# ShenhanQian/GaussianAvatars

Hardware: AMD Instinct MI355X
Metric: frames/sec fwd+bwd @100k SH-3 splats 802x550 (higher is better)
Workload: dtype f32; 1 GPU; BASELINE configs[2]: 100000 mesh-bound SH-3 splats (synthetic stand-in for media/306), 802x550 (HxW), select_mesh_by_timestep + render + L1-vs-white + backward, no optimiser step; splats=100000, width=550, height=802, sh_degree=3, scene=ellipsoid, splat_order=morton (io.spatial_sort: the loaders' default), num_rendered=2322054, num_binned=1851307, tile_culling=True, binding=fused, parallelism=one process, one GPU, 300 frames in turn; no collective

## Files before the change

gaussianavatars_amd/csrc/gsr_api.hip:

```cpp
#include <hip/hip_runtime.h>

#include <atomic>
#include <chrono>
#include <cstdarg>
#include <cstdio>
#include <cstdlib>
#include <cstring>
#include <map>
#include <mutex>
#include <tuple>
#include <thread>
#include <vector>

#include "gsr_device.h"


namespace {

thread_local char g_err[512] = "";

int fail(int code, const char* fmt, ...)
{
    va_list ap;
    va_start(ap, fmt);
// ... 488 lines not shown
    uint32_t* qpos = (uint32_t*)(b + bl.qpos);
    uint32_t* qcount = (uint32_t*)(b + bl.qcount);
    uint32_t* qstart = (uint32_t*)(b + bl.qstart);
    const bool write_lists = settings->tile_culling == 0 || settings->tile_culling == 2;
    uint32_t* qlist = (uint32_t*)(b + bl.qlist);

    if (prod) {
        const uint32_t nb = (uint32_t)bl.nb, chunks = (uint32_t)bl.chunks;
        const int Q = 4 * tiles;
        uint32_t* bcount = (uint32_t*)(b + bl.bcount);
        uint32_t* bstart = (uint32_t*)(b + bl.bstart);
        uint32_t* bcursor = (uint32_t*)(b + bl.bcursor);
        uint32_t* border = (uint32_t*)(b + bl.border);
        unsigned long long* dkeys = (unsigned long long*)(b + bl.dkeys);
        unsigned long long* dtmp = (unsigned long long*)(b + bl.dtmp);
        uint32_t* order = (uint32_t*)(b + bl.order);
        const uint32_t* brec_rect = (const uint32_t*)(g + gl.brec);
        {
            TIMED(GSR_K_DEPTH_SORT, stream);
            const int dblocks = pblocks < GSR_BIN_BLOCKS ? pblocks : GSR_BIN_BLOCKS;
            uint32_t* bhist = (uint32_t*)(b + bl.bhist);
            hipLaunchKernelGGL(gsr::k_dbucket, dim3(dblocks), dim3(256), (size_t)nb * 4, stream, P, brec_rect, (const float*)pa.depths, hdr, nb,
                               bcount, bhist);
            hipLaunchKernelGGL(gsr::k_dscan, dim3(1), dim3(1024), 0, stream, nb, (const uint32_t*)bcount, bstart, bcursor, border, hdr);
            hipLaunchKernelGGL(gsr::k_dscatter, dim3(dblocks), dim3(256), (size_t)nb * 4, stream, P, brec_rect, (const float*)pa.depths,
                               (const gsr::BinHeader*)hdr, nb, (const uint32_t*)bstart, bcursor, dkeys, (const uint32_t*)bhist);
            hipLaunchKernelGGL((gsr::k_dsort<GSR_SORT_SMALL_KEYS, 256>), dim3(nb), dim3(256), 0, stream, 0u, 0xFFFFFFFFu,
                               (const uint32_t*)border, (const uint32_t*)bcount, (const uint32_t*)bstart, dkeys, dtmp, order);
            KERNEL_CHECK("depth sort", stream, dbg);
        }
        gsr::QBinArgs qa;
        qa.Q = Q; qa.gx = gx; qa.chunks = chunks;
        qa.qmask = (unsigned long long*)(b + bl.qmask);
        qa.hdr = hdr; qa.brec = (const float4*)(g + gl.brec); qa.order = order;
        qa.qhist = (uint32_t*)(b + bl.qhist); qa.qprefix = (const uint32_t*)(b + bl.qprefix); qa.qstart = qstart; qa.qpos = qpos;
        qa.capacity = cap;
        const size_t count_lds = (((size_t)Q + 3) / 4) * 4;
        const size_t walk_lds = (size_t)Q * 4;
        if (walk_lds > 48 * 1024)
            if (int rc = ensure_dynamic_lds((const void*)gsr::k_qscatter, (size_t)walk_lds)) return rc;
        const int walk_blocks = (int)chunks;
        {
            TIMED(GSR_K_QCOUNT, stream);
            hipLaunchKernelGGL(gsr::k_qcount, dim3(walk_blocks), dim3(256), count_lds, stream, qa);
            KERNEL_CHECK("k_qcount", stream, dbg);
        }
        {
            TIMED(GSR_K_QSCAN, stream);
            hipLaunchKernelGGL(gsr::k_qscan, dim3(((Q + 3) / 4 + 31) / 32), dim3(1024), 0, stream, Q, chunks, (const uint8_t*)(b + bl.qhist),
                               (uint32_t*)(b + bl.qprefix), qcount);
            hipLaunchKernelGGL(gsr::k_qscan_glob, dim3(1), dim3(1024), 0, stream, tiles, (const uint32_t*)qcount, qstart, tile_order, hdr,
                               slot_dev, seq, post_cap);
            KERNEL_CHECK("k_qscan", stream, dbg);
        }
        {
            TIMED(GSR_K_QSCATTER, stream);
            hipLaunchKernelGGL(gsr::k_qscatter, dim3(walk_blocks), dim3(64), walk_lds, stream, qa);
            KERNEL_CHECK("k_qscatter", stream, dbg);
        }
    } else if (rankp) {
        const uint32_t nb = (uint32_t)bl.nb;
        const int bin_blocks = pblocks < GSR_RANK_BLOCKS ? pblocks : GSR_RANK_BLOCKS;
        const bool direct = gsr::rank_direct(gx, tiles);
        uint32_t* const chunk_bounds = reinterpret_cast<uint32_t*>((uint4*)(b + bl.pstat) + 5 * (size_t)pblocks);
        const size_t hist_bytes = direct ? 0 : (size_t)tiles * sizeof(uint32_t);
        const size_t count_lds = (size_t)nb * 4 + (direct ? 0 : (size_t)(gx + 1) * (size_t)(gy + 1) * sizeof(uint32_t));
        if (count_lds > 48 * 1024) {
            if (int rc = ensure_dynamic_lds((const void*)gsr::k_rcount, (size_t)count_lds)) return rc;
        }
        const bool one_band_lds = (int)bl.nbands <= 1;
        const size_t stage_bytes = GSR_RSCATTER_STAGE_BYTES(one_band_lds), hist_al = (hist_bytes + 15) & ~(size_t)15;
        static const bool balanced_on = [] { const char* e = getenv("GSR_RSCATTER_BALANCED"); return !(e && e[0] == '0'); }();
        const bool balanced = balanced_on && hist_al + stage_bytes + 20 * 1024 <= 160 * 1024;
        const int stage_off = balanced ? (int)hist_al : -1;
        const size_t scatter_lds = balanced ? hist_al + stage_bytes : hist_bytes;
        if (scatter_lds > 48 * 1024)
        {
            if (int rc = ensure_dynamic_lds((const void*)gsr::k_rsort_rscatter, scatter_lds)) return rc;
            if (int rc = ensure_dynamic_lds((const void*)gsr::k_rscatter<8>, scatter_lds)) return rc;
        }
        uint32_t* block_hist = (uint32_t*)(b + bl.block_hist);
        uint32_t* bcount = (uint32_t*)(b + bl.bcount);
        uint32_t* bstart = (uint32_t*)(b + bl.bstart);
        uint32_t* bcursor = (uint32_t*)(b + bl.bcursor);
        uint32_t* bhist = (uint32_t*)(b + bl.bhist);
        unsigned long long* dkeys = (unsigned long long*)(b + bl.dkeys);
        unsigned long long* dtmp = (unsigned long long*)(b + bl.dtmp);
        uint32_t* rank = (uint32_t*)(b + bl.rank);
        uint2* ranks = (uint2*)(b + bl.ranks);
        const int nbands = (int)bl.nbands;
        const float inv_band_rows = 1.0f / (float)bl.band_rows;
        uint2* obs = nbands > 1 ? (uint2*)(b + bl.obs) : nullptr;
        uint32_t* bandcnt = (uint32_t*)(b + bl.bandcnt);
        const uint32_t nwc = (uint32_t)(((size_t)P + GSR_RANK_BAND_CHUNK - 1) / GSR_RANK_BAND_CHUNK);
        gsr::BandTables bt;
        bt.nbands = (uint32_t)nbands;
        bt.inv_band_rows = inv_band_rows;
        bt.over = (const uint32_t*)(b + bl.rank_over);
        ushort4* srect = (ushort4*)(b + bl.srect);
        uint32_t* tile_start = (uint32_t*)(b + bl.tile_start);
        uint32_t* tile_cursor = (uint32_t*)(b + bl.tile_cursor);
        uint2* ranges = (uint2*)(b + bl.ranges);
        if (pblocks > 0) {
            TIMED(GSR_K_COUNT, stream);
            hipLaunchKernelGGL(gsr::k_rcount, dim3(bin_blocks), dim3(GSR_RANK_BIN_THREADS), count_lds, stream, rank_ilv, P, gx, tiles,
                               pblocks, nb, (const ushort4*)srect, (const uint32_t*)pa.tiles_touched,
                               (const float*)pa.depths, (const uint4*)pa.pstat, tile_count, rect_total, block_hist, bcount, bhist, hdr, chunk_bounds);
            KERNEL_CHECK("k_rcount", stream, dbg);
        }
        const bool one_band = nbands <= 1;
        {
            TIMED(GSR_K_DEPTH_SORT, stream);
            gsr::TileScanArgs ts;
            ts.tiles = tiles; ts.tile_count = tile_count; ts.tile_start = tile_start; ts.tile_cursor = tile_cursor; ts.ranges = ranges;
            ts.tile_order = tile_order; ts.tdesc = (uint4*)(b + bl.tdesc); ts.total_dev = total_dev; ts.mailbox = slot_dev; ts.seq = seq;
            ts.post_capacity = post_cap;
            ts.hdr = pblocks > 0 ? hdr : nullptr;
            hipLaunchKernelGGL(gsr::k_rdscatter, dim3((pblocks > 0 ? bin_blocks : 0) + 1), dim3(GSR_RANK_BIN_THREADS), (size_t)nb * 4, stream, rank_ilv, P, nb,
                               (const ushort4*)srect, (const float*)pa.depths, hdr, (const uint32_t*)bcount, bstart, bcursor, dkeys, (const uint32_t*)bhist, ts,
                               (const uint32_t*)chunk_bounds);
            KERNEL_CHECK("k_rdscatter", stream, dbg);
            if (!one_band && pblocks > 0) {
                hipLaunchKernelGGL(gsr::k_rdsort, dim3(nb), dim3(256), 0, stream, (const uint32_t*)bcount, (const uint32_t*)bstart, dkeys, dtmp, rank, obs,
                                   (const ushort4*)srect, (int)bl.band_rows);
                KERNEL_CHECK("k_rdsort", stream, dbg);
                const uint32_t wgs = (nwc + 3u) / 4u;
                hipLaunchKernelGGL(gsr::k_band_count, dim3(wgs), dim3(256), 0, stream, (const gsr::BinHeader*)hdr, (const uint2*)obs,
                                   (uint32_t)nbands, nwc, bandcnt);
                hipLaunchKernelGGL(gsr::k_band_scan, dim3(nbands), dim3(1024), 0, stream, hdr, nwc, bandcnt);
                hipLaunchKernelGGL(gsr::k_band_rank, dim3(wgs), dim3(256), 0, stream, (const gsr::BinHeader*)hdr, (const uint2*)obs,
                                   (uint32_t)nbands, nwc, (const uint32_t*)bandcnt, (uint4*)rank, (uint32_t*)(b + bl.rank_over));
                KERNEL_CHECK("k_band_rank", stream, dbg);
            }
        }
        if (pblocks > 0) {
            TIMED(GSR_K_SCATTER, stream);
            if (one_band) {
                hipLaunchKernelGGL(gsr::k_rsort_rscatter, dim3(bin_blocks + nb), dim3(GSR_RANK_BIN_THREADS), scatter_lds, stream, rank_ilv, bin_blocks, P, gx, tiles,
                                   (const ushort4*)srect, (const float4*)pa.sspan, (const uint32_t*)tile_start, tile_cursor, (uint32_t*)ranks, cap,
                                   (const unsigned long long*)total_dev, (const uint32_t*)block_hist, (const uint32_t*)bcount, (const uint32_t*)bstart,
                                   dkeys, dtmp, rank, stage_off, (const uint32_t*)chunk_bounds);
                KERNEL_CHECK("k_rsort_rscatter", stream, dbg);
            } else {
                hipLaunchKernelGGL(gsr::k_rscatter<8>, dim3(bin_blocks), dim3(GSR_RANK_BIN_THREADS), scatter_lds, stream, rank_ilv, P, gx, tiles, bt,
                                   (const ushort4*)srect, (const uint32_t*)rank, (const float4*)pa.sspan, (const uint32_t*)tile_start, tile_cursor, ranks, cap,
                                   (const unsigned long long*)total_dev, (const uint32_t*)block_hist, stage_off, (const uint32_t*)chunk_bounds);
                KERNEL_CHECK("k_rscatter", stream, dbg);
            }
        }
        {
            TIMED(GSR_K_TILE_SORT, stream);
            const size_t space = (size_t)P < (size_t)GSR_RANK_MAX_SPLATS ? (size_t)P : (size_t)GSR_RANK_MAX_SPLATS;
            const uint32_t words = (uint32_t)((space + 2047) / 2048) * 64u;
            hipLaunchKernelGGL(gsr::k_tile_rank, dim3(tiles), dim3(GSR_RANK_TILE_THREADS), (size_t)words * 6, stream, words, gx, nbands,
                               inv_band_rows, (const uint4*)(b + bl.tdesc), (const uint2*)ranks, one_band ? (const uint32_t*)rank : nullptr, (const float*)pa.depths,
                               (const gsr::BinHeader*)hdr, write_lists ? (unsigned long long*)(b + bl.keys) : nullptr,
                               (uint32_t*)(b + bl.point_list), write_lists ? qlist : nullptr, qpos, qcount, qstart,
                               cap, (const unsigned long long*)total_dev);
            KERNEL_CHECK("k_tile_rank", stream, dbg);
        }
    } else {
    const int bin_blocks = pblocks < GSR_BIN_BLOCKS ? pblocks : GSR_BIN_BLOCKS;
    uint32_t* block_hist = (uint32_t*)(b + bl.block_hist);
    const size_t hist_bytes = tiles > GSR_LDS_HIST_TILES ? 0 : (size_t)tiles * sizeof(uint32_t);
    if (hist_bytes > 48 * 1024) {
        if (int rc = ensure_dynamic_lds((const void*)gsr::k_count<false>, (size_t)hist_bytes)) return rc;
        if (int rc = ensure_dynamic_lds((const void*)gsr::k_count<true>, (size_t)hist_bytes)) return rc;
        if (int rc = ensure_dynamic_lds((const void*)gsr::k_scatter<false>, (size_t)hist_bytes)) return rc;
        if (int rc = ensure_dynamic_lds((const void*)gsr::k_scatter<true>, (size_t)hist_bytes)) return rc;
    }
    const bool cull = settings->tile_culling != 0;
    if (pblocks > 0) {
        TIMED(GSR_K_COUNT, stream);
        hipLaunchKernelGGL(cull ? gsr::k_count<true> : gsr::k_count<false>, dim3(bin_blocks), dim3(256), hist_bytes, stream, P, gx, tiles,
                           (const ushort4*)pa.rect, (const uint32_t*)pa.tiles_touched, (const float4*)pa.grec, tile_count, rect_total, block_hist);
        KERNEL_CHECK("k_count", stream, dbg);
    }
    uint32_t* tile_start = (uint32_t*)(b + bl.tile_start);
    uint32_t* tile_cursor = (uint32_t*)(b + bl.tile_cursor);
    uint2* ranges = (uint2*)(b + bl.ranges);
    {
        TIMED(GSR_K_TILE_SCAN, stream);
        hipLaunchKernelGGL(gsr::k_tile_scan, dim3(1), dim3(1024), 0, stream, tiles, (const uint32_t*)tile_count, tile_start, tile_cursor,
                           ranges, tile_order, total_dev, slot_dev, seq, post_cap);
        KERNEL_CHECK("k_tile_scan", stream, dbg);
    }

    unsigned long long* keys = (unsigned long long*)(b + bl.keys);
    uint32_t* point_list = (uint32_t*)(b + bl.point_list);
    if (pblocks > 0) {
        TIMED(GSR_K_SCATTER, stream);
        hipLaunchKernelGGL(cull ? gsr::k_scatter<true> : gsr::k_scatter<false>, dim3(bin_blocks), dim3(256), hist_bytes, stream, P, gx, tiles,
                           (const float*)pa.depths, (const ushort4*)pa.rect, (const uint32_t*)pa.tiles_touched, (const float4*)pa.grec,
                           (const uint32_t*)tile_start, tile_cursor, keys, cap, (const unsigned long long*)total_dev,
                           (const uint32_t*)block_hist);
        KERNEL_CHECK("k_scatter", stream, dbg);
    }
    {
        TIMED(GSR_K_TILE_SORT, stream);
        auto sort_class = [&](auto kernel, int threads, uint32_t n_lo, uint32_t n_hi) {
            hipLaunchKernelGGL(kernel, dim3(tiles), dim3(threads), 0, stream, n_lo, n_hi, gx, (const uint32_t*)tile_order,
                               (const uint32_t*)tile_count, (const uint32_t*)tile_start, keys, write_lists ? point_list : nullptr, write_lists ? qlist : nullptr, qpos, qcount, qstart,
                               (const float4*)pa.grec, cap,
                               (const unsigned long long*)total_dev);
        };
        sort_class(gsr::k_tile_sort<GSR_SORT_XL_KEYS, 1024>, 1024, (uint32_t)GSR_SORT_LDS_KEYS, 0xFFFFFFFFu);
        sort_class(gsr::k_tile_sort<GSR_SORT_LDS_KEYS, 1024>, 1024, (uint32_t)GSR_SORT_SMALL_KEYS, (uint32_t)GSR_SORT_LDS_KEYS);
        sort_class(gsr::k_tile_sort<GSR_SORT_SMALL_KEYS, 256>, 256, 0u, (uint32_t)GSR_SORT_SMALL_KEYS);
        KERNEL_CHECK("k_tile_sort", stream, dbg);
    }
    }
    {
        TIMED(GSR_K_RENDER, stream);
        static const int cont_grid = [] { const char* e = getenv("GSR_CONT_GRID"); const int v = e ? atoi(e) : 0; return v > 0 ? v : GSR_CONT_GRID_DEFAULT; }();
        const int cgrid = 4 * tiles < cont_grid ? 4 * tiles : cont_grid;
        const bool conts = ds.fast_blend && ds.cont_chunks > 0;
        if (!conts) ds.cont_chunks = 0;
        const bool infer = ds.forward_only && !conts;
        auto* const render_k = !ds.fast_blend ? (infer ? &gsr::k_render<false, 0, true> : &gsr::k_render<false, 0, false>)
                               : (conts && ds.cont_mode == 1 ? &gsr::k_render<true, 1, false> : (infer ? &gsr::k_render<true, 0, true> : &gsr::k_render<true, 0, false>));
#ifndef GSR_EXP_NO_SOLO
        const bool solo = !(conts && ds.cont_mode == 1);
#else
        const bool solo = false;
#endif
        hipLaunchKernelGGL(render_k, solo ? dim3(4 * tiles) : dim3(tiles + cgrid), dim3(solo ? 64 : 256), 0, stream, ds, (const uint32_t*)tile_order, (const uint32_t*)qstart,
                           (const uint32_t*)qcount, (const float4*)pa.grec, (const uint32_t*)qpos, write_lists ? (const uint32_t*)qlist : nullptr, (float*)(im + il.final_T), (uint32_t*)(im + il.n_contrib),
                           (uint32_t*)(im + il.n_contrib_q), (float*)(im + il.c_final), (float4*)(im + il.ck), out_color, cap,
                           (const unsigned long long*)total_dev, (uint32_t*)(im + il.units), tiles);
        KERNEL_CHECK("k_render", stream, dbg);
        if (conts && ds.cont_mode == 2) {
            hipLaunchKernelGGL((gsr::k_render<true, 2, false>), dim3(cgrid), dim3(64 * GSR_CONT_WAVES), 0, stream, ds, (const uint32_t*)tile_order, (const uint32_t*)qstart,
                               (const uint32_t*)qcount, (const float4*)pa.grec, (const uint32_t*)qpos, write_lists ? (const uint32_t*)qlist : nullptr, (float*)(im + il.final_T), (uint32_t*)(im + il.n_contrib),
                               (uint32_t*)(im + il.n_contrib_q), (float*)(im + il.c_final), (float4*)(im + il.ck), out_color, cap,
                               (const unsigned long long*)total_dev, (uint32_t*)(im + il.units), tiles);
            KERNEL_CHECK("k_render_cont", stream, dbg);
        }
    }

    if (deferred) {
        *num_rendered_host = -1;
        return GSR_OK;
    }
    const auto t0 = std::chrono::steady_clock::now();
    unsigned long long v;
    unsigned spins = 0;
    for (;;) {
        v = __atomic_load_n((unsigned long long*)slot, __ATOMIC_ACQUIRE);
        if (v != 0 && (v >> 40) == seq) break;
        if (++spins > 2000) {
            std::this_thread::yield();
            if ((spins & 0xFFF) == 0) {
                if (hipStreamQuery(stream) != hipErrorNotReady) {
                    v = __atomic_load_n((unsigned long long*)slot, __ATOMIC_ACQUIRE);
                    if (v != 0 && (v >> 40) == seq) break;
                    hipError_t e = hipStreamSynchronize(stream);
                    return fail(GSR_E_HIP, "stream finished without posting the instance count: %s", hipGetErrorString(e));
                }
                if (std::chrono::steady_clock::now() - t0 > std::chrono::seconds(120))
                    return fail(GSR_E_TIMEOUT, "timed out waiting for the instance count");
            }
        }
    }
    g_wait_ns.fetch_add((long long)std::chrono::duration_cast<std::chrono::nanoseconds>(std::chrono::steady_clock::now() - t0).count());
    g_waits.fetch_add(1);
    const int64_t I = (int64_t)(v & kCountMask);
    note_posted(GSR_COUNT_SLOTS, v);
    *num_rendered_host = I;
    if (I > 0xFFFFFFFFll) return fail(GSR_E_ARG, "%lld (splat, tile) instances exceed the 32-bit offsets of the binning state", (long long)I);
    if (I > binning_capacity) return fail(GSR_E_CAPACITY, "binning capacity %lld < %lld instances", (long long)binning_capacity, (long long)I);
    return GSR_OK;
}

int gsr_forward_ex(const GsrSettings* settings, int32_t P, int32_t M, const float* means3D, const float* shs, const float* shs_rest,
                   const float* colors_precomp, const float* opacities, const float* scales, const float* rotations,
                   const float* cov3D_precomp, float* out_color, int32_t* radii, void* geom, void* binning,
                   int64_t binning_capacity, void* img, int64_t* num_rendered_host, void* stream)
{
    return forward_impl(settings, P, M, means3D, shs, shs_rest, colors_precomp, opacities, scales, rotations, cov3D_precomp, out_color, radii,
                        geom, binning, binning_capacity, img, num_rendered_host, stream, nullptr);
}

int gsr_forward_bound(const GsrSettings* settings, int32_t P, int32_t M, const GsrBound* bound, const float* xyz_local, const float* shs,
                      const float* shs_rest, const float* opacity_logit, const float* log_scales, const float* rot_local,
                      float* out_color, int32_t* radii, void* geom, void* binning, int64_t binning_capacity, void* img,
                      int64_t* num_rendered_host, void* stream)
{
    if (!bound) return fail(GSR_E_ARG, "gsr_forward_bound: bound is NULL");
    return forward_impl(settings, P, M, xyz_local, shs, shs_rest, nullptr, opacity_logit, log_scales, rot_local, nullptr, out_color, radii,
                        geom, binning, binning_capacity, img, num_rendered_host, stream, bound);
}

int gsr_forward(const GsrSettings* settings, int32_t P, int32_t M, const float* means3D, const float* shs,
                const float* colors_precomp, const float* opacities, const float* scales, const float* rotations,
                const float* cov3D_precomp, float* out_color, int32_t* radii, void* geom, void* binning,
                int64_t binning_capacity, void* img, int64_t* num_rendered_host, void* stream)
{
    return gsr_forward_ex(settings, P, M, means3D, shs, nullptr, colors_precomp, opacities, scales, rotations, cov3D_precomp, out_color,
                          radii, geom, binning, binning_capacity, img, num_rendered_host, stream);
}

static int backward_impl(const GsrSettings* settings, int32_t P, int32_t M, const float* means3D, const float* shs, const float* shs_rest,
                         const float* colors_precomp, const float* scales, const float* rotations, const float* cov3D_precomp,
                         const int32_t* radii, void* geom, const void* binning, int64_t binning_capacity, const void* img,
                         int64_t num_rendered, const float* dL_dpix, float* dL_dmeans3D, float* dL_dmeans2D,
                         float* dL_dsh, float* dL_dsh_rest, float* dL_dcolors, float* dL_dopacity, float* dL_dscales, float* dL_drotations,
                         float* dL_dcov3D, void* stream_, const GsrBound* bound, const float* opacity_logit)
// ... 182 lines not shown
```

gaussianavatars_amd/csrc/gsr_device.h:

```cpp
#pragma once
#include <hip/hip_runtime.h>
#include <stdint.h>

#include "../../include/gsr.h"

#define GSR_WAVE 64
#define GSR_TILE_PIX (GSR_BLOCK_X * GSR_BLOCK_Y)
#define GSR_SORT_LDS_KEYS 8192
#define GSR_SORT_XL_KEYS 16384
#define GSR_SORT_SMALL_KEYS 2048
#define GSR_ACC_STRIDE 16
#define GSR_ACC64_STRIDE 10
#define GSR_FIXED_BITS 58
#define GSR_LDS_HIST_TILES 40960
#define GSR_RANK_MAX_BUCKETS 4096
#define GSR_RANK_HIST_TILES (GSR_LDS_HIST_TILES - GSR_RANK_MAX_BUCKETS)
#define GSR_RANK_BANDS 24
#define GSR_RANK_MAX_BANDS 32
#define GSR_RANK_BAND_CHUNK 256
#define GSR_RANK_IDX_BITS 28
#define GSR_RANK_MAX_SPLATS 262144
#define GSR_RANK_TILE_THREADS 512
#define GSR_RANK_WINDOW 4096
#ifndef GSR_RANK_GROUP
#define GSR_RANK_GROUP 16
#endif
#define GSR_RANK_BIN_THREADS 1024

#include "bind_math.h"

namespace gsr {

typedef float f32x8 __attribute__((ext_vector_type(8)));

struct Settings {
    int H, W;
    float tanfovx, tanfovy;
    float scale_modifier;
    int sh_degree;
    int exact_scale_grad;
    int forward_only;
    int deterministic;
    int fast_blend;
    int cont_chunks;
    int cont_mode;
    const float* __restrict__ bg;
    const float* __restrict__ viewmatrix;
    const float* __restrict__ projmatrix;
    const float* __restrict__ campos;
};

__device__ constexpr float kC0 = 0.28209479177387814f;
__device__ constexpr float kC1 = 0.4886025119029199f;
__device__ constexpr float kC2_0 = 1.0925484305920792f;
__device__ constexpr float kC2_1 = -1.0925484305920792f;
__device__ constexpr float kC2_2 = 0.31539156525252005f;
__device__ constexpr float kC2_3 = -1.0925484305920792f;
__device__ constexpr float kC2_4 = 0.5462742152960396f;
__device__ constexpr float kC3_0 = -0.5900435899266435f;
__device__ constexpr float kC3_1 = 2.890611442640554f;
__device__ constexpr float kC3_2 = -0.4570457994644658f;
__device__ constexpr float kC3_3 = 0.3731763325901154f;
__device__ constexpr float kC3_4 = -0.4570457994644658f;
__device__ constexpr float kC3_5 = 1.445305721320277f;
__device__ constexpr float kC3_6 = -0.5900435899266435f;

__device__ __forceinline__ float sel_min(float a, float b) { return a < b ? a : b; }
__device__ __forceinline__ float sel_max(float a, float b) { return a > b ? a : b; }

__device__ __forceinline__ float gsr_expf(float x)
{
    if (!(x > -87.0f)) return 0.0f;
    if (x > 88.0f) x = 88.0f;
    const float l2e_hi = 1.44269502162933349609375f;
    const float l2e_lo = 1.92596299112661746e-8f;
    const float n = __builtin_rintf(x * l2e_hi);
    float f = __builtin_fmaf(x, l2e_hi, -n);
    f = __builtin_fmaf(x, l2e_lo, f);
    float p = 1.52527338040598402800e-5f;
    p = __builtin_fmaf(p, f, 1.54035303933816099544e-4f);
    p = __builtin_fmaf(p, f, 1.33335581464284434234e-3f);
    p = __builtin_fmaf(p, f, 9.61812910762847716197e-3f);
    p = __builtin_fmaf(p, f, 5.55041086648215799532e-2f);
    p = __builtin_fmaf(p, f, 2.40226506959100712334e-1f);
    p = __builtin_fmaf(p, f, 6.93147180559945309417e-1f);
    p = __builtin_fmaf(p, f, 1.0f);
    return __builtin_ldexpf(p, (int)n);
}

__device__ __forceinline__ float gsr_expf_blend(float x)
{
    const float l2e_hi = 1.44269502162933349609375f;
    const float l2e_lo = 1.92596299112661746e-8f;
    const float n = __builtin_rintf(x * l2e_hi);
    float f = __builtin_fmaf(x, l2e_hi, -n);
    f = __builtin_fmaf(x, l2e_lo, f);
    float p = 1.52527338040598402800e-5f;
    p = __builtin_fmaf(p, f, 1.54035303933816099544e-4f);
    p = __builtin_fmaf(p, f, 1.33335581464284434234e-3f);
    p = __builtin_fmaf(p, f, 9.61812910762847716197e-3f);
    p = __builtin_fmaf(p, f, 5.55041086648215799532e-2f);
    p = __builtin_fmaf(p, f, 2.40226506959100712334e-1f);
    p = __builtin_fmaf(p, f, 6.93147180559945309417e-1f);
    p = __builtin_fmaf(p, f, 1.0f);
    return __builtin_ldexpf(p, (int)n);
}

__device__ __forceinline__ int f2i_sat(float v)
{
    if (v != v) return 0;
    if (v >= 2147483648.0f) return 2147483647;
    if (v <= -2147483648.0f) return (-2147483647 - 1);
    return (int)v;
}

__device__ __forceinline__ float ndc2pix(float v, int S)
{
    return (float)((((double)v + 1.0) * (double)S - 1.0) * 0.5);
}

__device__ __forceinline__ int lane_id() { return (int)__builtin_amdgcn_mbcnt_hi(~0u, __builtin_amdgcn_mbcnt_lo(~0u, 0u)); }

template <int CTRL, int ROW_MASK>
__device__ __forceinline__ float dpp_f(float v)
{
    return __int_as_float(__builtin_amdgcn_update_dpp(0, __float_as_int(v), CTRL, ROW_MASK, 0xf, false));
}
__device__ __forceinline__ float wave_sum_hi(float v)
{
    v += dpp_f<0xB1, 0xf>(v);
    v += dpp_f<0x4E, 0xf>(v);
    v += dpp_f<0x141, 0xf>(v);
    v += dpp_f<0x140, 0xf>(v);
    v += dpp_f<0x142, 0xa>(v);
    v += dpp_f<0x143, 0xc>(v);
    return v;
}
__device__ __forceinline__ uint32_t wave_max_u32(uint32_t v)
{
    auto mx = [](uint32_t a, uint32_t b) { return a > b ? a : b; };
    v = mx(v, (uint32_t)__builtin_amdgcn_update_dpp(0, (int)v, 0xB1, 0xf, 0xf, false));
    v = mx(v, (uint32_t)__builtin_amdgcn_update_dpp(0, (int)v, 0x4E, 0xf, 0xf, false));
    v = mx(v, (uint32_t)__builtin_amdgcn_update_dpp(0, (int)v, 0x141, 0xf, 0xf, false));
    v = mx(v, (uint32_t)__builtin_amdgcn_update_dpp(0, (int)v, 0x140, 0xf, 0xf, false));
    uint32_t a = (uint32_t)__builtin_amdgcn_readlane((int)v, 0);
    uint32_t b = (uint32_t)__builtin_amdgcn_readlane((int)v, 16);
    uint32_t c = (uint32_t)__builtin_amdgcn_readlane((int)v, 32);
    uint32_t d = (uint32_t)__builtin_amdgcn_readlane((int)v, 48);
    return mx(mx(a, b), mx(c, d));
}

__device__ __forceinline__ uint32_t wave_scan_incl_u32(uint32_t v)
{
    v += (uint32_t)__builtin_amdgcn_update_dpp(0, (int)v, 0x111, 0xf, 0xf, false);
    v += (uint32_t)__builtin_amdgcn_update_dpp(0, (int)v, 0x112, 0xf, 0xf, false);
    v += (uint32_t)__builtin_amdgcn_update_dpp(0, (int)v, 0x114, 0xf, 0xf, false);
    v += (uint32_t)__builtin_amdgcn_update_dpp(0, (int)v, 0x118, 0xf, 0xf, false);
    v += (uint32_t)__builtin_amdgcn_update_dpp(0, (int)v, 0x142, 0xa, 0xf, false);
    v += (uint32_t)__builtin_amdgcn_update_dpp(0, (int)v, 0x143, 0xc, 0xf, false);
    return v;
}

struct Reach {
    float px, py, A, B, C, tau, nBiC, nBiA;
    int mode;
};
__device__ __forceinline__ Reach reach_of(float px, float py, float A, float B, float C, float opacity)
{
    Reach r;
    r.px = px; r.py = py; r.A = A; r.B = B; r.C = C;
    r.tau = 0.f; r.nBiC = 0.f; r.nBiA = 0.f;
    if (!(opacity * 255.0f >= 1.0f)) { r.mode = 2; return r; }
    r.tau = logf(255.0f * opacity) * 1.0001f + 1e-3f;
    if (!(A > 0.f && C > 0.f && (A * C - B * B) > 0.f)) { r.mode = 1; return r; }
    r.nBiC = -B / C;
    r.nBiA = -B / A;
// ... 455 lines not shown
```

gaussianavatars_amd/csrc/gsr_rank.hip:

```cpp
#include "gsr_device.h"
#include "gsr_sort.h"

namespace gsr {

__device__ __forceinline__ uint32_t rank_bucket(float depth, float lo, float scale, uint32_t nb)
{
    const int b = f2i_sat((depth - lo) * scale);
    return (uint32_t)min(max(b, 0), (int)nb - 1);
}
__device__ __forceinline__ void rank_bucket_map(uint32_t dmin_bits, uint32_t dmax_bits, uint32_t nb, float& lo, float& scale)
{
    lo = __uint_as_float(dmin_bits);
    const float span = __uint_as_float(dmax_bits) - lo;
    scale = span > 0.f ? (float)nb * 0.99999f / span : 0.f;
}
__device__ __forceinline__ uint32_t wave_min_u32(uint32_t v) { return ~wave_max_u32(~v); }

template <int G = GSR_RANK_GROUP, typename F>
__device__ __forceinline__ void for_each_tile_grouped(int minx, int miny, int maxx, int maxy, uint32_t n, F f)
{
    constexpr uint32_t BIG = 256;
    const int lane = lane_id(), sub = lane & (G - 1);
    if (n > 0 && n <= BIG) {
        const uint32_t w = (uint32_t)(maxx - minx);
// ... 684 lines not shown
    }
    auto f4u = [](float4 v) { return make_uint4(__float_as_uint(v.x), __float_as_uint(v.y), __float_as_uint(v.z), __float_as_uint(v.w)); };
    auto emit = [&](uint32_t x, uint32_t y, const Span& b, const uint4& brk4, uint32_t bfb, uint32_t bidx) {
        const uint32_t tile = y * (uint32_t)gx + x;
        uint32_t brk = brk4.x;
        if (bands) {
            const uint32_t band = (uint32_t)(((float)y + 0.5f) * bt.inv_band_rows), k = band - bfb;
            brk = k == 0u ? brk4.x : k == 1u ? brk4.y : k == 2u ? brk4.z : brk4.w;
            if (k > 3u) brk = bt.over[(size_t)bidx * bt.nbands + band];
        }
        const uint32_t m = quadrant_mask_of(b, (float)(x * GSR_BLOCK_X), (float)(y * GSR_BLOCK_Y));
        const uint32_t slot = direct ? tile_start[tile] + atomicAdd(&tile_cursor[tile], 1u) : atomicAdd(&hist[tile], 1u);
        if (LEAN) lean[slot] = bidx | (m << GSR_RANK_IDX_BITS);
        else ranks[slot] = make_uint2(brk, bidx | (m << GSR_RANK_IDX_BITS));
    };
    for (int base = 0; base < chunk; base += stride) {
        const int i = mine_of(base);
        const In cur = nxt;
        nxt = fetch(mine_of(base + stride));
        const int minx = cur.q.x, miny = cur.q.y, maxx = cur.q.z, maxy = cur.q.w;
        const uint32_t n = (uint32_t)((maxx - minx) * (maxy - miny)), w = (uint32_t)(maxx - minx);
        const bool big = n > BIG;
        const uint32_t nbal = big ? 0u : n;
        const uint32_t incl = wave_scan_incl_u32(nbal), excl = incl - nbal;
        const uint32_t total = (uint32_t)__builtin_amdgcn_readlane((int)incl, 63);
        wave_lds_handover();
        rows[lane][0] = f4u(cur.s0);
        rows[lane][1] = f4u(cur.s1);
        if (!LEAN) rows[lane][2] = cur.rk;
        rows[lane][ROW - 1] = make_uint4((uint32_t)minx | (uint32_t)miny << 16, w, excl, (uint32_t)i);
        wave_lds_handover();
        uint32_t carry = 0u;
        for (uint32_t k0 = 0; k0 < total; k0 += 64u) {
            own[lane] = 0u;
            const uint32_t rel = excl - k0;
            if (nbal != 0u && rel < 64u) own[rel] = (uint32_t)lane + 1u;
            wave_lds_handover();
            uint32_t o = wave_scan_incl_max_u32(own[lane]);
            o = o > carry ? o : carry;
            carry = (uint32_t)__builtin_amdgcn_readlane((int)o, 63);
            const uint32_t k = k0 + (uint32_t)lane;
            if (k < total) {
                const uint4(&r)[ROW] = rows[o - 1u];
                const uint4 a0 = r[0], a1 = r[1], a3 = r[ROW - 1];
                uint4 brk4 = make_uint4(0u, 0u, 0u, 0u);
                if (!LEAN) brk4 = r[2];
                Span sp;
                sp.px = __uint_as_float(a0.x); sp.py = __uint_as_float(a0.y); sp.B = __uint_as_float(a0.z); sp.det = __uint_as_float(a0.w);
                sp.twoTA = __uint_as_float(a1.x); sp.A = __uint_as_float(a1.y); sp.dyr = __uint_as_float(a1.z); sp.mode = (int)a1.w;
                const uint32_t ominx = a3.x & 0xFFFFu, ominy = a3.x >> 16, ow = a3.y, t = k - a3.z;
                const uint32_t row = (uint32_t)(((float)t + 0.5f) * __builtin_amdgcn_rcpf((float)ow));
                const uint32_t fb = bands ? (uint32_t)(((float)ominy + 0.5f) * bt.inv_band_rows) : 0u;
                emit(ominx + t - row * ow, ominy + row, sp, brk4, fb, a3.w);
            }
        }
        uint64_t bigm = __ballot(big);
        if (bigm) {
            Span sp;
            sp.px = cur.s0.x; sp.py = cur.s0.y; sp.B = cur.s0.z; sp.det = cur.s0.w;
            sp.twoTA = cur.s1.x; sp.A = cur.s1.y; sp.dyr = cur.s1.z; sp.mode = __float_as_int(cur.s1.w);
            const uint32_t fb = bands ? (uint32_t)(((float)miny + 0.5f) * bt.inv_band_rows) : 0u;
            while (bigm) {
                const int src = __builtin_ctzll(bigm);
                bigm &= bigm - 1;
                auto bf = [&](float v) { return __int_as_float(__builtin_amdgcn_readlane(__float_as_int(v), src)); };
                auto bu = [&](uint32_t v) { return (uint32_t)__builtin_amdgcn_readlane((int)v, src); };
                Span b;
                b.px = bf(sp.px); b.py = bf(sp.py); b.B = bf(sp.B); b.det = bf(sp.det); b.twoTA = bf(sp.twoTA); b.A = bf(sp.A); b.dyr = bf(sp.dyr);
                b.mode = __builtin_amdgcn_readlane(sp.mode, src);
                const uint4 brk4 = make_uint4(bu(cur.rk.x), bu(cur.rk.y), bu(cur.rk.z), bu(cur.rk.w));
                const uint32_t bfb = bu(fb), bidx = bu((uint32_t)i), bminx = bu((uint32_t)minx), bminy = bu((uint32_t)miny), bw = bu(w), bn = bu(n);
                for (uint32_t k = (uint32_t)lane; k < bn; k += GSR_WAVE) emit(bminx + k % bw, bminy + k / bw, b, brk4, bfb, bidx);
            }
        }
    }
}

template <int G>
__global__ __launch_bounds__(GSR_RANK_BIN_THREADS) void k_rscatter(int ilv, int P, int gx, int tiles, BandTables bt, const ushort4* __restrict__ srect,
                                                                    const uint32_t* __restrict__ rank, const float4* __restrict__ sspan,
                                                                    const uint32_t* __restrict__ tile_start, uint32_t* __restrict__ tile_cursor,
                                                                    uint2* __restrict__ ranks, unsigned long long capacity,
                                                                    const unsigned long long* __restrict__ total_dev,
                                                                    const uint32_t* __restrict__ block_hist, int stage_off, const uint32_t* __restrict__ cb)
{
    extern __shared__ uint32_t dyn_lds[];
    if (stage_off >= 0)
        rscatter_balanced<false>(*reinterpret_cast<RscatterStage<false>*>(reinterpret_cast<unsigned char*>(dyn_lds) + stage_off), P, gx, tiles, bt, srect, rank, sspan,
                                 tile_start, tile_cursor, ranks, capacity, total_dev, block_hist, (int)gridDim.x, ilv, cb);
    else
        rscatter_body<G, false>(P, gx, tiles, bt, srect, rank, sspan, tile_start, tile_cursor, ranks, capacity, total_dev, block_hist, (int)gridDim.x, ilv, cb);
}

__global__ __launch_bounds__(GSR_RANK_BIN_THREADS) void k_rsort_rscatter(int ilv, int scatter_blocks, int P, int gx, int tiles, const ushort4* __restrict__ srect,
                                                                          const float4* __restrict__ sspan, const uint32_t* __restrict__ tile_start,
                                                                          uint32_t* __restrict__ tile_cursor, uint32_t* __restrict__ entries,
                                                                          unsigned long long capacity, const unsigned long long* __restrict__ total_dev,
                                                                          const uint32_t* __restrict__ block_hist, const uint32_t* __restrict__ bcount,
                                                                          const uint32_t* __restrict__ bstart, unsigned long long* __restrict__ dkeys,
                                                                          unsigned long long* __restrict__ dtmp, uint32_t* __restrict__ rank, int stage_off,
                                                                          const uint32_t* __restrict__ cb)
{
    extern __shared__ uint32_t dyn_lds[];
    if ((int)blockIdx.x < scatter_blocks) {
        BandTables bt;
        bt.nbands = 1u; bt.inv_band_rows = 1.f; bt.over = nullptr;
        if (stage_off >= 0)
            rscatter_balanced<true>(*reinterpret_cast<RscatterStage<true>*>(reinterpret_cast<unsigned char*>(dyn_lds) + stage_off), P, gx, tiles, bt, srect, nullptr,
                                    sspan, tile_start, tile_cursor, reinterpret_cast<uint2*>(entries), capacity, total_dev, block_hist, scatter_blocks, ilv, cb);
        else
            rscatter_body<GSR_RANK_GROUP, true>(P, gx, tiles, bt, srect, nullptr, sspan, tile_start, tile_cursor, reinterpret_cast<uint2*>(entries), capacity,
                                                total_dev, block_hist, scatter_blocks, ilv, cb);
        return;
    }
    if (threadIdx.x >= 256) return;
    __shared__ unsigned long long skeys[GSR_SORT_SMALL_KEYS];
    depth_sort_bucket(blockIdx.x - (uint32_t)scatter_blocks, bcount, bstart, dkeys, dtmp, rank, nullptr, nullptr, 1, skeys);
}

template __global__ void k_rscatter<8>(int, int, int, int, BandTables, const ushort4*, const uint32_t*, const float4*, const uint32_t*, uint32_t*, uint2*, unsigned long long,
                                       const unsigned long long*, const uint32_t*, int, const uint32_t*);

template <int THREADS>
__device__ __forceinline__ void tile_streams(uint32_t total, uint32_t n, uint32_t tile, uint32_t start, uint32_t* __restrict__ sorted,
                                             const uint32_t* __restrict__ lsorted, uint32_t (*__restrict__ cntw)[GSR_RANK_WINDOW / 64 + 1],
                                             const float* __restrict__ depths, unsigned long long* __restrict__ keys,
                                             uint32_t* __restrict__ qpbase, uint32_t* __restrict__ qlbase, uint32_t* __restrict__ qcount)
{
    constexpr int NW = THREADS / 64, EPT = GSR_RANK_WINDOW / THREADS, NE = EPT * NW;
    static_assert(NE == GSR_RANK_WINDOW / 64 && NE <= 64, "one (chunk, wave) counter per lane in the scan");
    static_assert(EPT % 4 == 0, "four chunks at a time");
    const int tid = threadIdx.x, lane = tid & 63, wid = tid >> 6;
    const bool fast = lsorted != nullptr;
    const unsigned long long tile_hi = (unsigned long long)tile << 32;
    uint32_t run[4] = {0u, 0u, 0u, 0u};
    for (uint32_t win_lo = 0; win_lo < total; win_lo += (uint32_t)GSR_RANK_WINDOW) {
        const uint32_t m = min((uint32_t)GSR_RANK_WINDOW, total - win_lo);
        const uint32_t i0 = win_lo;
        uint32_t msk[EPT], rnk[EPT], sid[EPT];
#pragma unroll
        for (int h = 0; h < EPT / 4; ++h) {
            if ((uint32_t)(4 * h * THREADS) >= m) {
#pragma unroll
                for (int k = 0; k < 4; ++k) {
                    msk[4 * h + k] = 0u; rnk[4 * h + k] = 0u; sid[4 * h + k] = 0u;
                    if (lane < 4) cntw[lane][(4 * h + k) * NW + wid] = 0u;
                }
                continue;
            }
            uint32_t ent[4];
#pragma unroll
            for (int k = 0; k < 4; ++k) {
                const uint32_t j = (uint32_t)(4 * h + k) * THREADS + (uint32_t)tid;
                ent[k] = j < m ? (fast ? lsorted[j] : sorted[i0 + j]) : 0u;
            }
#pragma unroll
            for (int k = 0; k < 4; ++k) {
                const int c = 4 * h + k;
                const uint32_t j = (uint32_t)c * THREADS + (uint32_t)tid;
                const uint32_t idx = ent[k] & ((1u << GSR_RANK_IDX_BITS) - 1u);
                if (j < m && keys) {
                    keys[start + i0 + j] = tile_hi | (unsigned long long)__float_as_uint(depths[idx]);
                    sorted[i0 + j] = idx;
                }
                const uint32_t mq = j < m ? ent[k] >> GSR_RANK_IDX_BITS : 0u;
                msk[c] = mq;
                sid[c] = idx;
                uint32_t r = 0;
#pragma unroll
                for (int q = 0; q < 4; ++q) {
                    const unsigned long long bal = __ballot((mq >> q) & 1u);
                    r |= (uint32_t)__builtin_amdgcn_mbcnt_hi((uint32_t)(bal >> 32), __builtin_amdgcn_mbcnt_lo((uint32_t)bal, 0u)) << (8 * q);
                    if (lane == 0) cntw[q][c * NW + wid] = (uint32_t)__builtin_popcountll(bal);
                }
                rnk[c] = r;
            }
        }
        __syncthreads();
        if (wid < 4) {
            const uint32_t a = lane < NE ? cntw[wid][lane] : 0u;
            const uint32_t incl = wave_scan_incl_u32(a);
            if (lane < NE) cntw[wid][lane] = incl - a;
            if (lane == 63) cntw[wid][NE] = incl;
        }
        __syncthreads();
#pragma unroll
        for (int c = 0; c < EPT; ++c) {
            const uint32_t mq = msk[c];
            if (mq) {
                const uint32_t j = (uint32_t)c * THREADS + (uint32_t)tid;
#pragma unroll
                for (int q = 0; q < 4; ++q) {
                    if ((mq >> q) & 1u) {
                        const uint32_t pos = run[q] + cntw[q][c * NW + wid] + ((rnk[c] >> (8 * q)) & 0xFFu);
                        qpbase[(size_t)q * n + pos] = sid[c];
                        if (qlbase) qlbase[(size_t)q * n + pos] = i0 + j;
                    }
                }
            }
        }
#pragma unroll
        for (int q = 0; q < 4; ++q) run[q] += cntw[q][NE];
        __syncthreads();
    }
    if (tid < 4) qcount[4 * tile + tid] = tid == 0 ? run[0] : tid == 1 ? run[1] : tid == 2 ? run[2] : run[3];
}

__global__ __launch_bounds__(GSR_RANK_TILE_THREADS) void k_tile_rank(uint32_t words, int gx, int nbands, float inv_band_rows,
                                                    const uint4* __restrict__ tdesc, const uint2* __restrict__ ranks, const uint32_t* __restrict__ rank_of,
                                                    const float* __restrict__ depths, const BinHeader* __restrict__ hdr,
                                                    unsigned long long* __restrict__ keys, uint32_t* __restrict__ point_list,
                                                    uint32_t* __restrict__ qlist, uint32_t* __restrict__ qpos, uint32_t* __restrict__ qcount,
                                                    uint32_t* __restrict__ qstart, unsigned long long capacity,
                                                    const unsigned long long* __restrict__ total_dev)
{
    constexpr int THREADS = GSR_RANK_TILE_THREADS, NW = THREADS / 64, EPT = GSR_RANK_WINDOW / THREADS, NE = EPT * NW;
    constexpr int ROWS = GSR_RANK_MAX_SPLATS / 2048, RPL = (ROWS + 63) / 64;
#ifndef GSR_RANK_UB
#define GSR_RANK_UB 8
#endif
    constexpr int UB = GSR_RANK_UB;
    static_assert(NE <= 64, "one (chunk, wave) counter per lane in the epilogue's scan");
    static_assert(EPT % 4 == 0, "the epilogue gathers four chunks at a time");
    extern __shared__ uint32_t bitmap[];
    uint16_t* const wprefix = reinterpret_cast<uint16_t*>(bitmap + words);
    __shared__ uint32_t cntw[4][NE + 1];
    __shared__ uint32_t rowoff[ROWS + 1];
    __shared__ uint32_t lsorted[UB * THREADS];
    if (*total_dev > capacity) return;
    const uint4 td = tdesc[blockIdx.x];
    const uint32_t tile = td.x, n = td.y;
    const int tid = threadIdx.x, lane = tid & 63, wid = tid >> 6;
    if (n == 0) {
        if (tid < 4) { qcount[4 * tile + tid] = 0u; qstart[4 * tile + tid] = 0u; }
        return;
    }
    const uint32_t start = td.z;
    if (tid < 4) qstart[4 * tile + tid] = 4u * start + (uint32_t)tid * n;
    const uint2* __restrict__ rk2 = ranks + start;
    const uint32_t* __restrict__ rk1 = reinterpret_cast<const uint32_t*>(ranks) + start;
    auto entry = [&](uint32_t i) {
        if (!rank_of) return rk2[i];
        const uint32_t e = rk1[i];
        return make_uint2(rank_of[e & ((1u << GSR_RANK_IDX_BITS) - 1u)], e);
    };
    uint32_t* const qpbase = qpos + (size_t)4 * start;
    uint32_t* const qlbase = qlist ? qlist + (size_t)4 * start : nullptr;
    const uint32_t space = nbands > 1 ? hdr->band_total[(uint32_t)(((float)(tile / (uint32_t)gx) + 0.5f) * inv_band_rows)] : hdr->nvis;
    const uint32_t per_pass = words * 32u;
    const bool single = space <= per_pass;
    const bool fast = single && n <= (uint32_t)(UB * THREADS);
    uint32_t* const sorted = point_list + start;

    uint2 e0[UB];
#pragma unroll
    for (int k = 0; k < UB; ++k) {
        const uint32_t i = (uint32_t)(k * THREADS + tid);
        e0[k] = i < n ? entry(i) : make_uint2(0xFFFFFFFFu, 0u);
    }
    auto pass = [&](const uint32_t lo, const uint32_t span, const bool in_lds, const uint32_t placed) {
        const uint32_t rows = (((span + 31u) >> 5) + 63u) >> 6;
        for (uint32_t w = tid; w < rows * 64u; w += THREADS) bitmap[w] = 0u;
        __syncthreads();
#pragma unroll
        for (int k = 0; k < UB; ++k) {
            const uint32_t r = e0[k].x - lo;
            if (r < span) atomicOr(&bitmap[r >> 5], 1u << (r & 31u));
        }
        for (uint32_t base = UB * THREADS; base < n; base += UB * THREADS) {
            uint32_t r[UB];
#pragma unroll
            for (int k = 0; k < UB; ++k) {
                const uint32_t i = base + (uint32_t)(k * THREADS + tid);
                r[k] = i < n ? entry(i).x - lo : 0xFFFFFFFFu;
            }
#pragma unroll
            for (int k = 0; k < UB; ++k)
                if (r[k] < span) atomicOr(&bitmap[r[k] >> 5], 1u << (r[k] & 31u));
        }
        __syncthreads();
        for (uint32_t row = wid; row < rows; row += NW) {
            const uint32_t w = row * 64u + (uint32_t)lane;
            const uint32_t v = (uint32_t)__builtin_popcount(bitmap[w]);
            const uint32_t incl = wave_scan_incl_u32(v);
            wprefix[w] = (uint16_t)(incl - v);
            if (lane == 63) rowoff[row] = incl;
        }
        __syncthreads();
        if (wid == 0) {
            uint32_t a[RPL], sum = 0;
#pragma unroll
            for (int j = 0; j < RPL; ++j) {
                const uint32_t rr = (uint32_t)(RPL * lane + j);
                a[j] = rr < rows ? rowoff[rr] : 0u;
                sum += a[j];
            }
            const uint32_t incl = wave_scan_incl_u32(sum);
            uint32_t acc = incl - sum;
#pragma unroll
            for (int j = 0; j < RPL; ++j) {
                const uint32_t rr = (uint32_t)(RPL * lane + j);
                if (rr < rows) rowoff[rr] = acc;
                acc += a[j];
            }
            if (lane == 63) rowoff[ROWS] = incl;
        }
        __syncthreads();
        auto position = [&](uint32_t r) {
            const uint32_t w = r >> 5;
            return rowoff[w >> 6] + (uint32_t)wprefix[w] + (uint32_t)__builtin_popcount(bitmap[w] & ((1u << (r & 31u)) - 1u));
        };
        if (in_lds) {
#pragma unroll
            for (int k = 0; k < UB; ++k) {
                const uint32_t r = e0[k].x - lo;
                if (r < span) lsorted[position(r)] = e0[k].y;
            }
        } else {
            for (uint32_t base = 0; base < n; base += UB * THREADS) {
                uint2 e[UB];
#pragma unroll
                for (int k = 0; k < UB; ++k) {
                    const uint32_t i = base + (uint32_t)(k * THREADS + tid);
                    e[k] = i < n ? entry(i) : make_uint2(0xFFFFFFFFu, 0u);
                }
#pragma unroll
                for (int k = 0; k < UB; ++k) {
                    const uint32_t r = e[k].x - lo;
                    if (r < span) sorted[placed + position(r)] = e[k].y;
                }
            }
        }
        return rowoff[ROWS];
    };
    uint32_t placed = 0;
    if (single) {
        placed = pass(0u, space, fast, 0u);
    } else {
        for (uint32_t lo = 0; lo < space; lo += per_pass) {
            placed += pass(lo, min(per_pass, space - lo), false, placed);
            __syncthreads();
        }
    }
    __syncthreads();
    tile_streams<THREADS>(placed, n, tile, start, sorted, fast ? lsorted : nullptr, cntw, depths, keys, qpbase, qlbase, qcount);
}

}
```

Before: 3822 frames/s.

## Alias tile-rank sorted staging onto bitmap LDS and batch rank loads

The static lsorted LDS buffer in k_tile_rank is removed and aliased onto the dynamic bitmap region. The dynamic allocation grows to cover whichever of the two is larger, and an extra barrier separates computing positions from writing. Rank loads are batched with clamped indices so all gathers are issued before use. The bitmap is cleared with 16-byte stores, and the per-row popcount scans are batched four rows at a time. Together these aim to cut LDS footprint and raise occupancy and memory-level parallelism in the per-tile ranking kernel, at the cost of an added __syncthreads and the early-exit path now reading tdesc before returning.

```diff
diff --git a/gaussianavatars_amd/csrc/gsr_api.hip b/gaussianavatars_amd/csrc/gsr_api.hip
--- a/gaussianavatars_amd/csrc/gsr_api.hip
+++ b/gaussianavatars_amd/csrc/gsr_api.hip
@@ -664,7 +664,8 @@
             TIMED(GSR_K_TILE_SORT, stream);
             const size_t space = (size_t)P < (size_t)GSR_RANK_MAX_SPLATS ? (size_t)P : (size_t)GSR_RANK_MAX_SPLATS;
             const uint32_t words = (uint32_t)((space + 2047) / 2048) * 64u;
-            hipLaunchKernelGGL(gsr::k_tile_rank, dim3(tiles), dim3(GSR_RANK_TILE_THREADS), (size_t)words * 6, stream, words, gx, nbands,
+            const size_t rank_lds = std::max((size_t)words * 6, (size_t)GSR_RANK_UB * GSR_RANK_TILE_THREADS * 4);
+            hipLaunchKernelGGL(gsr::k_tile_rank, dim3(tiles), dim3(GSR_RANK_TILE_THREADS), rank_lds, stream, words, gx, nbands,
                                inv_band_rows, (const uint4*)(b + bl.tdesc), (const uint2*)ranks, one_band ? (const uint32_t*)rank : nullptr, (const float*)pa.depths,
                                (const gsr::BinHeader*)hdr, write_lists ? (unsigned long long*)(b + bl.keys) : nullptr,
                                (uint32_t*)(b + bl.point_list), write_lists ? qlist : nullptr, qpos, qcount, qstart,
diff --git a/gaussianavatars_amd/csrc/gsr_device.h b/gaussianavatars_amd/csrc/gsr_device.h
--- a/gaussianavatars_amd/csrc/gsr_device.h
+++ b/gaussianavatars_amd/csrc/gsr_device.h
@@ -20,8 +20,15 @@
 #define GSR_RANK_BAND_CHUNK 256
 #define GSR_RANK_IDX_BITS 28
 #define GSR_RANK_MAX_SPLATS 262144
+#ifndef GSR_RANK_TILE_THREADS
 #define GSR_RANK_TILE_THREADS 512
+#endif
+#ifndef GSR_RANK_WINDOW
 #define GSR_RANK_WINDOW 4096
+#endif
+#ifndef GSR_RANK_UB
+#define GSR_RANK_UB 8
+#endif
 #ifndef GSR_RANK_GROUP
 #define GSR_RANK_GROUP 16
 #endif
diff --git a/gaussianavatars_amd/csrc/gsr_rank.hip b/gaussianavatars_amd/csrc/gsr_rank.hip
--- a/gaussianavatars_amd/csrc/gsr_rank.hip
+++ b/gaussianavatars_amd/csrc/gsr_rank.hip
@@ -860,7 +860,7 @@
 #pragma unroll
             for (int k = 0; k < 4; ++k) {
                 const uint32_t j = (uint32_t)(4 * h + k) * THREADS + (uint32_t)tid;
-                ent[k] = j < m ? (fast ? lsorted[j] : sorted[i0 + j]) : 0u;
+                ent[k] = j < m ? (fast ? lsorted[i0 + j] : sorted[i0 + j]) : 0u;
             }
 #pragma unroll
             for (int k = 0; k < 4; ++k) {
@@ -924,51 +924,59 @@
 {
     constexpr int THREADS = GSR_RANK_TILE_THREADS, NW = THREADS / 64, EPT = GSR_RANK_WINDOW / THREADS, NE = EPT * NW;
     constexpr int ROWS = GSR_RANK_MAX_SPLATS / 2048, RPL = (ROWS + 63) / 64;
-#ifndef GSR_RANK_UB
-#define GSR_RANK_UB 8
-#endif
     constexpr int UB = GSR_RANK_UB;
     static_assert(NE <= 64, "one (chunk, wave) counter per lane in the epilogue's scan");
     static_assert(EPT % 4 == 0, "the epilogue gathers four chunks at a time");
-    extern __shared__ uint32_t bitmap[];
+    extern __shared__ __align__(16) uint32_t bitmap[];
     uint16_t* const wprefix = reinterpret_cast<uint16_t*>(bitmap + words);
+    uint32_t* const lsorted = bitmap;
     __shared__ uint32_t cntw[4][NE + 1];
     __shared__ uint32_t rowoff[ROWS + 1];
-    __shared__ uint32_t lsorted[UB * THREADS];
-    if (*total_dev > capacity) return;
     const uint4 td = tdesc[blockIdx.x];
+    const bool over = *total_dev > capacity;
     const uint32_t tile = td.x, n = td.y;
     const int tid = threadIdx.x, lane = tid & 63, wid = tid >> 6;
-    if (n == 0) {
-        if (tid < 4) { qcount[4 * tile + tid] = 0u; qstart[4 * tile + tid] = 0u; }
+    if (over || n == 0) {
+        if (!over && tid < 4) { qcount[4 * tile + tid] = 0u; qstart[4 * tile + tid] = 0u; }
         return;
     }
     const uint32_t start = td.z;
-    if (tid < 4) qstart[4 * tile + tid] = 4u * start + (uint32_t)tid * n;
     const uint2* __restrict__ rk2 = ranks + start;
     const uint32_t* __restrict__ rk1 = reinterpret_cast<const uint32_t*>(ranks) + start;
-    auto entry = [&](uint32_t i) {
-        if (!rank_of) return rk2[i];
-        const uint32_t e = rk1[i];
-        return make_uint2(rank_of[e & ((1u << GSR_RANK_IDX_BITS) - 1u)], e);
+    auto load_batch = [&](const uint32_t base, uint2 (&e)[UB]) {
+        if (rank_of) {
+            uint32_t raw[UB];
+#pragma unroll
+            for (int k = 0; k < UB; ++k) raw[k] = rk1[min(base + (uint32_t)(k * THREADS + tid), n - 1u)];
+#pragma unroll
+            for (int k = 0; k < UB; ++k) {
+                const uint32_t r = rank_of[raw[k] & ((1u << GSR_RANK_IDX_BITS) - 1u)];
+                e[k] = base + (uint32_t)(k * THREADS + tid) < n ? make_uint2(r, raw[k]) : make_uint2(0xFFFFFFFFu, 0u);
+            }
+        } else {
+#pragma unroll
+            for (int k = 0; k < UB; ++k) {
+                const uint32_t i = base + (uint32_t)(k * THREADS + tid);
+                const uint2 v = rk2[min(i, n - 1u)];
+                e[k] = i < n ? v : make_uint2(0xFFFFFFFFu, 0u);
+            }
+        }
     };
     uint32_t* const qpbase = qpos + (size_t)4 * start;
     uint32_t* const qlbase = qlist ? qlist + (size_t)4 * start : nullptr;
-    const uint32_t space = nbands > 1 ? hdr->band_total[(uint32_t)(((float)(tile / (uint32_t)gx) + 0.5f) * inv_band_rows)] : hdr->nvis;
+    uint32_t* const sorted = point_list + start;
+
+    uint2 e0[UB];
+    load_batch(0u, e0);
+    if (tid < 4) qstart[4 * tile + tid] = 4u * start + (uint32_t)tid * n;
+    const uint32_t space = nbands > 1
+        ? hdr->band_total[__builtin_amdgcn_readfirstlane((uint32_t)(((float)(tile / (uint32_t)gx) + 0.5f) * inv_band_rows))] : hdr->nvis;
     const uint32_t per_pass = words * 32u;
     const bool single = space <= per_pass;
     const bool fast = single && n <= (uint32_t)(UB * THREADS);
-    uint32_t* const sorted = point_list + start;
-
-    uint2 e0[UB];
-#pragma unroll
-    for (int k = 0; k < UB; ++k) {
-        const uint32_t i = (uint32_t)(k * THREADS + tid);
-        e0[k] = i < n ? entry(i) : make_uint2(0xFFFFFFFFu, 0u);
-    }
     auto pass = [&](const uint32_t lo, const uint32_t span, const bool in_lds, const uint32_t placed) {
         const uint32_t rows = (((span + 31u) >> 5) + 63u) >> 6;
-        for (uint32_t w = tid; w < rows * 64u; w += THREADS) bitmap[w] = 0u;
+        for (uint32_t w4 = tid; w4 < rows * 16u; w4 += THREADS) reinterpret_cast<uint4*>(bitmap)[w4] = make_uint4(0u, 0u, 0u, 0u);
         __syncthreads();
 #pragma unroll
         for (int k = 0; k < UB; ++k) {
@@ -976,23 +984,32 @@
             if (r < span) atomicOr(&bitmap[r >> 5], 1u << (r & 31u));
         }
         for (uint32_t base = UB * THREADS; base < n; base += UB * THREADS) {
-            uint32_t r[UB];
+            uint2 e[UB];
+            load_batch(base, e);
 #pragma unroll
             for (int k = 0; k < UB; ++k) {
-                const uint32_t i = base + (uint32_t)(k * THREADS + tid);
-                r[k] = i < n ? entry(i).x - lo : 0xFFFFFFFFu;
-            }
-#pragma unroll
-            for (int k = 0; k < UB; ++k)
-                if (r[k] < span) atomicOr(&bitmap[r[k] >> 5], 1u << (r[k] & 31u));
-        }
-        __syncthreads();
-        for (uint32_t row = wid; row < rows; row += NW) {
-            const uint32_t w = row * 64u + (uint32_t)lane;
-            const uint32_t v = (uint32_t)__builtin_popcount(bitmap[w]);
-            const uint32_t incl = wave_scan_incl_u32(v);
-            wprefix[w] = (uint16_t)(incl - v);
-            if (lane == 63) rowoff[row] = incl;
+                const uint32_t r = e[k].x - lo;
+                if (r < span) atomicOr(&bitmap[r >> 5], 1u << (r & 31u));
+            }
+        }
+        __syncthreads();
+        for (uint32_t row0 = wid; row0 < rows; row0 += 4u * NW) {
+            uint32_t v[4], incl[4];
+#pragma unroll
+            for (int j = 0; j < 4; ++j) {
+                const uint32_t row = row0 + (uint32_t)j * NW;
+                v[j] = row < rows ? (uint32_t)__builtin_popcount(bitmap[row * 64u + (uint32_t)lane]) : 0u;
+            }
+#pragma unroll
+            for (int j = 0; j < 4; ++j) incl[j] = wave_scan_incl_u32(v[j]);
+#pragma unroll
+            for (int j = 0; j < 4; ++j) {
+                const uint32_t row = row0 + (uint32_t)j * NW;
+                if (row < rows) {
+                    wprefix[row * 64u + (uint32_t)lane] = (uint16_t)(incl[j] - v[j]);
+                    if (lane == 63) rowoff[row] = incl[j];
+                }
+            }
         }
         __syncthreads();
         if (wid == 0) {
@@ -1019,19 +1036,20 @@
             return rowoff[w >> 6] + (uint32_t)wprefix[w] + (uint32_t)__builtin_popcount(bitmap[w] & ((1u << (r & 31u)) - 1u));
         };
         if (in_lds) {
+            uint32_t pos[UB];
 #pragma unroll
             for (int k = 0; k < UB; ++k) {
                 const uint32_t r = e0[k].x - lo;
-                if (r < span) lsorted[position(r)] = e0[k].y;
-            }
+                pos[k] = r < span ? position(r) : 0xFFFFFFFFu;
+            }
+            __syncthreads();
+#pragma unroll
+            for (int k = 0; k < UB; ++k)
+                if (pos[k] != 0xFFFFFFFFu) lsorted[pos[k]] = e0[k].y;
         } else {
             for (uint32_t base = 0; base < n; base += UB * THREADS) {
                 uint2 e[UB];
-#pragma unroll
-                for (int k = 0; k < UB; ++k) {
-                    const uint32_t i = base + (uint32_t)(k * THREADS + tid);
-                    e[k] = i < n ? entry(i) : make_uint2(0xFFFFFFFFu, 0u);
-                }
+                load_batch(base, e);
 #pragma unroll
                 for (int k = 0; k < UB; ++k) {
                     const uint32_t r = e[k].x - lo;
```

Result: no change. 3846 frames/s, median of 6 (+0.6%).
